# Huangying-Zhan/DF-VO

Measured on AMD Instinct MI355X. Metric: KITTI-odom frames/sec (DF-VO per-pair tracking hot path: monodepth2 + LiteFlowNet fwd/bwd + kp selection + E/H RANSAC + scale), higher is better.
Workload: dtype f32 (f16x3 split products: two f16 planes per operand = 22 mantissa bits, three exact products per term, fp32 accumulate; direct one- / two-channel heads exact fp32)

## Files before the change

### df-vo_amd/capi.py

```python
import ctypes as C
import os

import numpy as np

from . import LIB_PATH


ITER_NOT_RUN = 3
PUSH_NO_FLOW = 1
ERR_RANGE = -4
ERR_EMPTY_SELECTION = -5
ERR_NO_CONSENSUS = -6


class DfvoError(RuntimeError):
    code = None


_lib = None


class Pose2d2dCfg(C.Structure):
    _fields_ = [("fx", C.c_double), ("cx", C.c_double), ("cy", C.c_double), ("reproj_thre", C.c_double),
                ("repeat", C.c_int), ("max_iters", C.c_int), ("KinvT", C.c_double * 9), ("Kinv", C.c_double * 9),
# ... 150 lines not shown
    "dfvo_vis_create": (_i, [_i, _i, C.POINTER(_vp)]),
    "dfvo_vis_destroy": (None, [_vp]),
    "dfvo_vis_cell_rect": (_i, [_vp, _i, _ip]),
    "dfvo_vis_draw_flow": (_i, [_vp, _i, _vp, _i, _i, C.POINTER(C.c_longlong)]),
    "dfvo_vis_draw_map": (_i, [_vp, _i, _vp, _i, _i, _i, _i, _i, _d, C.POINTER(_d)]),
    "dfvo_vis_draw_session": (_i, [_vp, _vp, C.c_longlong, _i, _d, _i, _d, C.POINTER(C.c_longlong), C.POINTER(_d)]),
    "dfvo_vis_session_cells": (_i, [_vp, C.c_longlong, _ip]),
    "dfvo_vis_clear_cell": (_i, [_vp, _i]),
    "dfvo_vis_fetch": (_i, [_vp, _i, _vp]),
    "dfvo_vis_counters": (_i, [_vp, C.POINTER(C.c_longlong)]),
    "dfvo_vis_device_ms": (_i, [_vp, C.POINTER(_f)]),
    "dfvo_vis_flow_rgb": (_i, [_vp, _vp, _i, _i, _vp, C.POINTER(C.c_longlong)]),
    "dfvo_vis_disparity_percentile90": (_i, [_vp, _vp, _i, _i, C.POINTER(_d)]),
    "dfvo_set_conv_precision": (_i, [C.c_char_p]),
    "dfvo_get_conv_precision": (C.c_char_p, []),
    "dfvo_set_sklearn_compat": (_i, [C.c_char_p]),
    "dfvo_f16s_overflow_count": (_i, [C.POINTER(C.c_ulonglong), _i]),
    "dfvo_set_fp32_winograd": (_i, [_i]),
    "dfvo_get_fp32_winograd": (_i, []),
    "dfvo_fp32_winograd_launches": (_i, [C.POINTER(C.c_ulonglong), _i]),
    "dfvo_conv_profile_begin": (_i, []),
    "dfvo_conv_profile_end": (_i, [_vp, _vp, _vp]),
    "dfvo_conv_profile_end_bytes": (_i, [_vp, _vp, _vp, _vp]),
    "dfvo_correlation": (_i, [_vp, _vp, _i, _i, _i, _i, _i, _f, _vp, _vp]),
    "dfvo_backward_warp": (_i, [_vp, _vp, _f, _i, _i, _i, _i, _vp, _vp, _vp, _vp]),
    "dfvo_warp_view": (_i, [_vp, _i, _i, _i, _vp, _i, _i, _f, _i, _i, _i, _i, _vp, _vp, _vp, _i, _i, _i, _i, _vp]),
    "dfvo_correlation_view": (_i, [_vp, _i, _i, _vp, _i, _i, _i, _i, _i, _i, _i, _i, _f, _vp, _i, _vp]),
    "dfvo_flow_mean": (_i, [_vp, _i, _i, _i, _i, _vp, _vp]),
    "dfvo_reg_prep": (_i, [_vp, _vp, _i, _i, _f, _vp, _i, _i, _i, _vp, _vp, _vp, _vp]),
    "dfvo_reg_head": (_i, [_vp, _i, _i, _vp, _i, _i, _vp, _f, _vp, _f, _i, _i, _i, _vp, _i, _i, _vp]),
# ... 202 lines not shown
```

### df-vo_amd/csrc/capi.hip

```cpp
#include "../../include/dfvo_hip.h"

#include <cstdlib>
#include <cstring>
#include <map>
#include <mutex>
#include <utility>
#include <vector>

#include "nets.h"
#include "ops.h"
#include "resize_lanczos.h"
#include "capi_types.h"

namespace dfvo {
static thread_local std::string g_err;
void set_last_error(const std::string& s) { g_err = s; }
const char* last_error() { return g_err.c_str(); }

int ensure_dyn_lds(const void* kernel, size_t bytes) {
    static std::mutex mu;
    static std::map<std::pair<int, const void*>, size_t> configured;
    int dev = 0;
    DFVO_HIP_CHECK(hipGetDevice(&dev));
    std::lock_guard<std::mutex> lock(mu);
// ... 96 lines not shown
    L.ksteps = ksteps;
    L.act = d->act;
    L.act_param = d->act_param;
    static DevArr<float>* const conv2d_ws = new DevArr<float>();
    static std::mutex conv2d_mu;
    std::lock_guard<std::mutex> conv2d_lock(conv2d_mu);
    if (!conv2d_ws->p) (void)conv2d_ws->alloc_zeroed((size_t)4 << 20);
    int rc = run_conv(L, d->N, d->H, d->W, View{d_src0, d->cs0, d->co0}, d->up0, View{d_src1, d->cs1, d->co1}, d_res,
                      d->res_cs, d->res_co, d_dst, d->dst_cs, d->dst_co, d->dst_zero_to, s, nullptr,
                      conv2d_ws->p ? conv2d_ws : nullptr);
    return finish(rc, s);
}

int dfvo_set_conv_precision(const char* name) { return conv_set_precision(name); }
const char* dfvo_get_conv_precision(void) { return conv_get_precision(); }
int dfvo_f16s_overflow_count(unsigned long long* h_count, int reset) { return conv_f16s_overflow_count(h_count, reset); }
int dfvo_set_fp32_winograd(int mode) { return conv_set_fp32_winograd(mode); }
int dfvo_get_fp32_winograd(void) { return conv_fp32_winograd_mode(); }
int dfvo_fp32_winograd_launches(unsigned long long* h_count, int reset) { return conv_fp32_winograd_launches(h_count, reset); }

int dfvo_conv_profile_begin(void) {
    conv_profile_begin();
    return DFVO_OK;
}
int dfvo_conv_profile_end(double* h_ms19, double* h_flops19, int* h_launches19) {
    DFVO_ARG_CHECK(h_ms19 && h_flops19 && h_launches19, "dfvo_conv_profile_end: null argument");
    return conv_profile_end(h_ms19, h_flops19, h_launches19);
}
int dfvo_conv_profile_end_bytes(double* h_ms24, double* h_flops24, int* h_launches24, double* h_bytes24) {
    DFVO_ARG_CHECK(h_ms24 && h_flops24 && h_launches24 && h_bytes24, "dfvo_conv_profile_end_bytes: null argument");
// ... 435 lines not shown
```

### df-vo_amd/csrc/conv.h

```cpp
#pragma once
#include <initializer_list>
#include <string>
#include <type_traits>
#include <vector>

#include "dfvo_common.h"

namespace dfvo {

enum Act { ACT_NONE = 0, ACT_LEAKY = 1, ACT_RELU = 2, ACT_ELU = 3, ACT_SIGMOID = 4 };
enum PadMode { PAD_ZERO = 0, PAD_REFLECT = 1 };

struct ConvParams {
    int N, H, W;
    int Ho, Wo;
    int kh, kw, stride, pad_h, pad_w;
    int pad_mode;
    const float* src0;
    int G0, cs0, co0, up0;
    const float* src1;
    int G1, cs1, co1;
    const float* wp;
    const float* bias;
    const float* wh;
// ... 46 lines not shown
    return (uint32_t)ky | ((uint32_t)kx << 5) | ((uint32_t)valid << 10) | ((uint32_t)src << 11) | ((uint32_t)choff << 16);
}
void conv_build_f16g_table(int c0, int c1, int kh, int kw, std::vector<uint32_t>* tab);
size_t conv_pack_weights_f16g(const float* w_oihw, int cout, int c0, int c1, int kh, int kw, const float* fold_scale,
                              unsigned short* out);
size_t conv_pack_weights_f32g(const float* w_oihw, int cout, int c0, int c1, int kh, int kw, const float* fold_scale, float* out);
size_t conv_wino_f32_weight_floats(int cout, int c0, int c1);
void conv_pack_weights_wino_f32(const float* w_oihw, int cout, int c0, int c1, const float* fold_scale, float* out);
unsigned long long conv_f16s_weights_clamped(bool reset);

constexpr int CONV_NUM_CFGS = 24;
int launch_conv(const ConvParams& p, hipStream_t stream, bool wino_all = false);
bool conv_wino_rule_may_accept(int cout, long long max_pixels);
struct RingShape { bool tc2; int ksp; };
RingShape ring_shape(long long M, int nblk, int steps);

int launch_igemm_f32(const ConvParams& p, hipStream_t stream, int bm, int bn);
int launch_win_f32(const ConvParams& p, hipStream_t stream, int cfg_id);
int launch_head_f32(const ConvParams& p, hipStream_t stream);
bool conv_f16s_ok(const ConvParams& p);
int launch_f16_window(const ConvParams& p, hipStream_t stream);
bool conv_f16g_ok(const ConvParams& p);
int launch_f16g(const ConvParams& p, hipStream_t stream);
unsigned* conv_f16s_overflow_counter();
int conv_f16s_overflow_count(unsigned long long* n, int reset);
bool conv_taps_f16s_ok(const ConvParams& p);
int launch_taps_f16s(const ConvParams& p, hipStream_t stream);
bool conv_f32g_ok(const ConvParams& p);
int launch_f32g(const ConvParams& p, hipStream_t stream);
int conv_fp32_winograd_mode();
// ... 49 lines not shown
```

### df-vo_amd/csrc/conv_dispatch.hip

```cpp
#include "conv.h"

namespace dfvo {

int conv_pick_bn(int cout, long long) {
    if (cout <= 16) return 16;
    if (cout <= 32) return 32;
    if (cout % 128 == 0) return 128;
    if (cout % 64 == 0) return 64;
    if (cout % 32 == 0) return 32;
    return 64;
}

static bool conv_use_head(const ConvParams& p) {
    if (p.cout > 2 || !p.wh) return false;
    if (p.kh != p.kw || p.stride != 1 || p.pad_h != p.kh / 2 || p.pad_w != p.kw / 2) return false;
    if (p.kh != 3 && p.kh != 5 && p.kh != 7) return false;
    return (long long)p.N * p.Ho * p.Wo >= 1024;
}

static bool conv_use_window(const ConvParams& p, int bn) {
    if (p.kh != p.kw || p.stride != 1 || p.pad_h != p.kh / 2 || p.pad_w != p.kw / 2) return false;
    const long long M = (long long)p.N * p.Ho * p.Wo;
    if (p.kh == 3) return bn >= 32 && M >= 30000;
    return (p.kh == 5 || p.kh == 7) && bn == 16 && (p.G0 + p.G1) >= 4 && M >= 8000;
// ... 28 lines not shown
    if (conv_use_head(p) || conv_use_window(p, bn)) return false;
    return (long long)p.N * p.Ho * p.Wo <= 8192;
}

RingShape ring_shape(long long M, int nblk, int steps) {
    const long long mblocks = (M + 31) / 32;
    const long long target = 2048;
    bool tc2 = (nblk % 2) == 0;
    if (tc2 && mblocks * (nblk / 2) * 8 * 2 < target && steps >= 64) tc2 = false;
    const long long tiles = mblocks * (tc2 ? nblk / 2 : nblk);
    int ksp = 1;
    while (ksp < (tc2 ? 8 : 16) && tiles * ksp * 2 <= target && steps >= 4 * ksp * 2) ksp *= 2;
    return {tc2, ksp};
}

int launch_conv(const ConvParams& p, hipStream_t stream, bool wino_all) {
    const long long M = (long long)p.N * p.Ho * p.Wo;
    const int bn = conv_pick_bn(p.cout, M);
    DFVO_ARG_CHECK(p.cout_pad % bn == 0, "launch_conv: cout_pad not a multiple of the N tile");
    DFVO_ARG_CHECK((p.cs0 % 4) == 0 && (p.co0 % 4) == 0, "launch_conv: src0 stride/offset must be multiples of 4");
    DFVO_ARG_CHECK(p.G1 == 0 || ((p.cs1 % 4) == 0 && (p.co1 % 4) == 0), "launch_conv: src1 stride/offset");
    if (conv_use_head(p)) return launch_head_f32(p, stream);
    if (p.wf16 && conv_f16s_ok(p)) return launch_f16_window(p, stream);
    if (conv_f16g_ok(p)) return launch_f16g(p, stream);
    if (conv_wino_applicable(p) && (wino_all || conv_wino_size_rule(p, bn))) return launch_wino(p, stream, conv_window_cfg(p, bn));
    if (conv_f32g_ok(p) && conv_f32g_takes(p, bn)) return launch_f32g(p, stream);
    if (conv_use_window(p, bn)) return launch_win_f32(p, stream, p.kh == 7 ? 16 : (p.kh == 5 ? 17 : conv_window_cfg(p, bn)));
    return launch_igemm_f32(p, stream, conv_pick_bm(p, bn), bn);
}

// ... 2 lines not shown
```

### df-vo_amd/csrc/conv_gemm_f16s.h

```cpp
#pragma once
#include "conv_epi.h"
#include "conv_f16_clamp.h"

namespace dfvo {

typedef unsigned int u32x4 __attribute__((ext_vector_type(4)));
typedef __attribute__((address_space(4))) const u32x4 cu32x4;

template <int WP, int KSP, int TC, int PF = 3, bool RAG = false, int NP = 3>
__global__ __launch_bounds__(64 * WP * KSP) void conv_gemm_f16s_kernel(const ConvParams p) {
    extern __shared__ __attribute__((aligned(16))) float f16g_red[];

    const int t = threadIdx.x, lane = t & 63;
    const int wave = __builtin_amdgcn_readfirstlane(t >> 6);
    const int wp = wave / KSP, wk = wave % KSP;
    const int lp = lane & 31, kb = lane >> 5;
    const int M = p.N * p.Ho * p.Wo;
    const int nb = gridDim.x;
    int bid = blockIdx.x;
    {
        const int q = nb >> 3, r = nb & 7, xcd = bid & 7, k = bid >> 3;
        bid = (xcd < r ? xcd * (q + 1) : r * (q + 1) + (xcd - r) * q) + k;
    }
    const int ny = p.wf16g_cout_pad / (32 * TC);
    const int ytile = bid % ny;
    bid /= ny;
    const int m = (bid * WP + wp) * 32 + lp;
    const bool vm = m < M;
    int iy0, ix0, nimg;
    {
        const int mm = vm ? m : 0;
        nimg = mm / (p.Ho * p.Wo);
        const int rem = mm - nimg * (p.Ho * p.Wo);
        const int oy = rem / p.Wo, ox = rem - oy * p.Wo;
        iy0 = oy * p.stride - p.pad_h;
        ix0 = ox * p.stride - p.pad_w;
    }
    const int n0 = ytile * (32 * TC);
    const int S = p.f16g_steps;
    const int per = (S + KSP - 1) / KSP;
    const int s0 = wk * per < S ? wk * per : S;
    const int s1 = s0 + per < S ? s0 + per : S;

    auto pin = [](int v) { return __builtin_amdgcn_readfirstlane(v); };
    auto pin64 = [](unsigned long long v) {
        const unsigned lo = __builtin_amdgcn_readfirstlane((unsigned)v), hi = __builtin_amdgcn_readfirstlane((unsigned)(v >> 32));
        return ((unsigned long long)hi << 32) | lo;
    };
    const cu32x4* const tab = (const cu32x4*)pin64((unsigned long long)p.f16g_tab);
    const unsigned long long src0 = pin64((unsigned long long)p.src0), src1 = pin64((unsigned long long)(p.G1 ? p.src1 : p.src0));
    const int cs0 = pin(p.cs0), cs1 = pin(p.cs1), co0 = pin(p.co0), co1 = pin(p.co1), up0 = pin(p.up0);
    const int H = pin(p.H), W = pin(p.W), refl = pin(p.pad_mode == PAD_REFLECT ? 1 : 0);
    const int H0 = H >> up0, W0 = W >> up0;
    const unsigned short* const wbase = p.wf16g + ((size_t)n0 * 32 + (kb * 32 + lp) * 8);
    const size_t w_step_stride = (size_t)pin(p.wf16g_cout_pad) * 32;

    f32x4 ra[PF][2];
    unsigned rav = 0;
    h16x8 rw[PF][TC][2];
    const bool fast_addr = !refl && up0 == 0;
    int* const gtab = reinterpret_cast<int*>(f16g_red + (KSP > 1 ? WP * KSP * TC * 16 * 64 : 0));
    if (fast_addr) {
        for (int i = t; i < S * 4; i += 64 * WP * KSP) {
            const unsigned e = p.f16g_tab[i];
            const int ky = e & 31, kx = (e >> 5) & 31;
            const bool s1e = ((e >> 11) & 1u) != 0;
            gtab[2 * i] = (ky * W + kx) * (s1e ? cs1 : cs0) + (int)(e >> 16);
            gtab[2 * i + 1] = (int)(e & 0xfffu);
        }
        __syncthreads();
// ... 168 lines not shown
        if (!vm) continue;
        if (fastq) {
            f32x4 x = v + b + r;
#pragma unroll
            for (int e = 0; e < 4; ++e) x[e] = apply_act(x[e], p.act, p.act_param);
            *reinterpret_cast<f32x4*>(p.dst + (size_t)m * p.dst_cs + p.dst_co + col0) = x;
        } else {
            conv_epilogue_quad(p, (size_t)m, col0, v, vec_ok);
        }
    }
}

template <int WP, int KSP, int TC, int PF = 3, bool RAG = false>
static int launch_f16g_cfg(const ConvParams& p, hipStream_t stream, int cfg_id) {
    const long long M = (long long)p.N * p.Ho * p.Wo;
    dim3 grid((unsigned)(((M + 32 * WP - 1) / (32 * WP)) * (p.wf16g_cout_pad / (32 * TC))), 1, 1);
    const bool fast_addr = p.pad_mode != PAD_REFLECT && p.up0 == 0;
    const size_t lds = (KSP > 1 ? (size_t)WP * KSP * TC * 16 * 64 * sizeof(float) : 0) + (fast_addr ? (size_t)p.f16g_steps * 32 : 0);
    return with_f16_terms(p, [&](auto np) -> int {
        const auto kernel = conv_gemm_f16s_kernel<WP, KSP, TC, PF, RAG, decltype(np)::value>;
        if (lds > 48 * 1024)
            if (int rc_lds = ensure_dyn_lds((const void*)kernel, lds)) return rc_lds;
        ConvProfScope prof(p, stream, cfg_id);
        hipLaunchKernelGGL(kernel, grid, dim3(64 * WP * KSP), lds, stream, p);
        DFVO_HIP_CHECK(hipGetLastError());
        static const std::string variant = conv_variant_name("f16g", {WP, KSP, TC}, RAG ? "rag" : nullptr);
        return prof.done((int)grid.x, TC, KSP * 100 + 1, variant.c_str(), decltype(np)::value);
    });
}

}
```

### df-vo_amd/csrc/conv_gemm_f32g.hip

```cpp
#include "conv.h"
#include "conv_epi.h"

namespace dfvo {

typedef float f32x16g __attribute__((ext_vector_type(16)));
typedef unsigned int u32x4g __attribute__((ext_vector_type(4)));
typedef __attribute__((address_space(4))) const u32x4g cu32x4g;

template <int WP, int KSP, int TC, int PF = 3>
__global__ __launch_bounds__(64 * WP * KSP) void conv_gemm_f32g_kernel(const ConvParams p) {
    extern __shared__ __attribute__((aligned(16))) float f32g_red[];

    const int t = threadIdx.x, lane = t & 63;
    const int wave = __builtin_amdgcn_readfirstlane(t >> 6);
    const int wp = wave / KSP, wk = wave % KSP;
    const int lp = lane & 31, kb = lane >> 5;
    const int M = p.N * p.Ho * p.Wo;
    const int nb = gridDim.x;
    int bid = blockIdx.x;
    {
        const int q = nb >> 3, r = nb & 7, xcd = bid & 7, k = bid >> 3;
        bid = (xcd < r ? xcd * (q + 1) : r * (q + 1) + (xcd - r) * q) + k;
    }
    const int ny = p.wf16g_cout_pad / (32 * TC);
    const int ytile = bid % ny;
    bid /= ny;
    const int m = (bid * WP + wp) * 32 + lp;
    const bool vm = m < M;
    int iy0, ix0, nimg;
    {
        const int mm = vm ? m : 0;
        nimg = mm / (p.Ho * p.Wo);
        const int rem = mm - nimg * (p.Ho * p.Wo);
        const int oy = rem / p.Wo, ox = rem - oy * p.Wo;
        iy0 = oy * p.stride - p.pad_h;
        ix0 = ox * p.stride - p.pad_w;
    }
    const int n0 = ytile * (32 * TC);
    const int S = p.f16g_steps;
    const int per = (S + KSP - 1) / KSP;
    const int s0 = wk * per < S ? wk * per : S;
    const int s1 = s0 + per < S ? s0 + per : S;
// ... 125 lines not shown
            for (int e = 0; e < 4; ++e) x[e] = apply_act(x[e], p.act, p.act_param);
            *reinterpret_cast<f32x4*>(p.dst + (size_t)m * p.dst_cs + p.dst_co + col0) = x;
        } else {
            conv_epilogue_quad(p, (size_t)m, col0, v, vec_ok);
        }
    }
}

bool conv_f32g_ok(const ConvParams& p) {
    return p.wf32g && p.f16g_tab && p.kh <= 31 && p.kw <= 31;
}

template <int WP, int KSP, int TC>
static int launch_f32g_cfg(const ConvParams& p, hipStream_t stream) {
    const long long M = (long long)p.N * p.Ho * p.Wo;
    dim3 grid((unsigned)(((M + 32 * WP - 1) / (32 * WP)) * (p.wf16g_cout_pad / (32 * TC))), 1, 1);
    const size_t lds = KSP > 1 ? (size_t)WP * KSP * TC * 16 * 64 * sizeof(float) : 0;
    if (lds > 48 * 1024)
        if (int rc_lds = ensure_dyn_lds((const void*)conv_gemm_f32g_kernel<WP, KSP, TC>, lds)) return rc_lds;
    ConvProfScope prof(p, stream, KSP == 1 ? 22 : 23);
    hipLaunchKernelGGL((conv_gemm_f32g_kernel<WP, KSP, TC>), grid, dim3(64 * WP * KSP), lds, stream, p);
    DFVO_HIP_CHECK(hipGetLastError());
    static const std::string variant = conv_variant_name("f32g", {WP, KSP, TC});
    return prof.done((int)grid.x, 0, KSP * 100 + 1, variant.c_str());
}

int launch_f32g(const ConvParams& p, hipStream_t stream) {
    const auto [tc2, ksp] = ring_shape((long long)p.N * p.Ho * p.Wo, p.wf16g_cout_pad / 32, p.f16g_steps);
    if (tc2) {
        switch (ksp) {
            case 1: return launch_f32g_cfg<4, 1, 2>(p, stream);
            case 2: return launch_f32g_cfg<2, 2, 2>(p, stream);
            case 4: return launch_f32g_cfg<1, 4, 2>(p, stream);
            default: return launch_f32g_cfg<1, 8, 2>(p, stream);
        }
    }
    switch (ksp) {
        case 1: return launch_f32g_cfg<4, 1, 1>(p, stream);
        case 2: return launch_f32g_cfg<2, 2, 1>(p, stream);
// ... 8 lines not shown
```

### df-vo_amd/csrc/conv_igemm_f32.hip

```cpp
#include "conv.h"

#include <algorithm>

#include "conv_epi.h"

namespace dfvo {

__device__ __forceinline__ void splitk_store(float* dst, f32x4 v) {
    union {
        float f[4];
        unsigned long long u[2];
    } c;
#pragma unroll
    for (int e = 0; e < 4; ++e) c.f[e] = v[e];
    __hip_atomic_store(reinterpret_cast<unsigned long long*>(dst), c.u[0], __ATOMIC_RELAXED, __HIP_MEMORY_SCOPE_AGENT);
    __hip_atomic_store(reinterpret_cast<unsigned long long*>(dst) + 1, c.u[1], __ATOMIC_RELAXED, __HIP_MEMORY_SCOPE_AGENT);
}
__device__ __forceinline__ f32x4 splitk_load(const float* src) {
    union {
        float f[4];
        unsigned long long u[2];
    } c;
    c.u[0] = __hip_atomic_load(reinterpret_cast<const unsigned long long*>(src), __ATOMIC_RELAXED, __HIP_MEMORY_SCOPE_AGENT);
    c.u[1] = __hip_atomic_load(reinterpret_cast<const unsigned long long*>(src) + 1, __ATOMIC_RELAXED, __HIP_MEMORY_SCOPE_AGENT);
// ... 48 lines not shown
    constexpr int BM = WM * TM * 16;
    constexpr int BN = WN * TN * 16;
    constexpr int A_CNT = (BM * 4 + 255) / 256;
    constexpr int B_CNT = (BN * 4 + 255) / 256;
    constexpr int TILE = BM * 16 + BN * 16;
    static_assert(WM * WN == 4, "4 waves per block");
    __shared__ __attribute__((aligned(16))) float lds[2 * TILE];
    __shared__ KGroup ktab[MAX_KGROUPS];

    const int t = threadIdx.x;
    const int lane = t & 63;
    const int wave = t >> 6;
    const int wm = wave / WN;
    const int wn = wave % WN;

    const int nb = gridDim.x;
    int bid = blockIdx.x;
    {
        const int q = nb >> 3, r = nb & 7, xcd = bid & 7, k = bid >> 3;
        bid = (xcd < r ? xcd * (q + 1) : r * (q + 1) + (xcd - r) * q) + k;
    }
    const int m0 = bid * BM;
    const int n0 = blockIdx.y * BN;
    const int M = p.N * p.Ho * p.Wo;
    const int G = p.G0 + p.G1;
    const int taps = p.kh * p.kw;
    const int per = (p.ksteps + (int)gridDim.z - 1) / (int)gridDim.z;
    const int s_begin = (int)blockIdx.z * per;
    const int s_end = s_begin + per < p.ksteps ? s_begin + per : p.ksteps;

    for (int g = s_begin * 4 + t; g < s_end * 4; g += 256) {
        const int tap = g / G;
        const int cg = g - tap * G;
        const int ky = tap / p.kw, kx = tap - ky * p.kw;
        KGroup e;
        const uint32_t valid = tap < taps ? 1u : 0u;
// ... 146 lines not shown
    constexpr int BN = WN * TN * 16;
    constexpr int WIN = WH * WW * PS;
    constexpr int BT = BN * 16;
    constexpr int W_ITEMS = WH * WW * 4;
    constexpr int W_CNT = (W_ITEMS + 255) / 256;
    constexpr int B_CNT = (BN * 4 + 255) / 256;
    static_assert(WM * WN == 4, "4 waves per block");
    __shared__ __attribute__((aligned(16))) float lds[2 * WIN + 2 * BT];
    float* const win = lds;
    float* const bst = lds + 2 * WIN;

    const int t = threadIdx.x, lane = t & 63, wave = t >> 6;
    const int wm = wave / WN, wn = wave % WN;
    const int li = lane & 15, kq = lane >> 4;
    const int tiles_x = (p.Wo + TW - 1) / TW, tiles_y = (p.Ho + TH - 1) / TH;
    const int nb = gridDim.x;
    int bid = blockIdx.x;
    {
        const int q = nb >> 3, r = nb & 7, xcd = bid & 7, k = bid >> 3;
        bid = (xcd < r ? xcd * (q + 1) : r * (q + 1) + (xcd - r) * q) + k;
    }
    const int n = bid / (tiles_y * tiles_x);
    const int trem = bid - n * (tiles_y * tiles_x);
    const int ty0 = (trem / tiles_x) * TH, tx0 = (trem % tiles_x) * TW;
    const int n0 = blockIdx.y * BN;
    const int G = p.G0 + p.G1;
    const int nchunk0 = (p.G0 + 3) >> 2, nchunk1 = (p.G1 + 3) >> 2, nchunks = nchunk0 + nchunk1;
    const int cper = (nchunks + (int)gridDim.z - 1) / (int)gridDim.z;
    const int c_begin = (int)blockIdx.z * cper;
    const int c_end = c_begin + cper < nchunks ? c_begin + cper : nchunks;

    int w_off0[W_CNT], w_off1[W_CNT], w_lds[W_CNT];
    bool w_ok[W_CNT];
#pragma unroll
    for (int r = 0; r < W_CNT; ++r) {
        const int id = t + 256 * r;
// ... 175 lines not shown
    p.dst[(size_t)m * p.dst_cs + p.dst_co + col] = v;
}

typedef __attribute__((address_space(4))) const f32x4 cf32x4;
typedef float f32x2 __attribute__((ext_vector_type(2)));
template <int KS, int CO, int PY = 2>
__global__ __launch_bounds__(256) void conv_head_f32_kernel(const ConvParams p) {
    constexpr int TW = 16, TH = 16 * PY, WH = TH + KS - 1, WW = TW + KS - 1, PS = 12;
    constexpr int WIN = WH * WW * PS;
    constexpr int W_ITEMS = WH * WW * 2;
    constexpr int W_CNT = (W_ITEMS + 255) / 256;
    constexpr int NR = PY + KS - 1;
    __shared__ __attribute__((aligned(16))) float win[WIN];
    const int t = threadIdx.x, tx = t & 15, ty = t >> 4;
    const int tiles_x = (p.Wo + TW - 1) / TW, tiles_y = (p.Ho + TH - 1) / TH;
    const int nb = gridDim.x;
    int bid = blockIdx.x;
    {
        const int q = nb >> 3, r = nb & 7, xcd = bid & 7, k = bid >> 3;
        bid = (xcd < r ? xcd * (q + 1) : r * (q + 1) + (xcd - r) * q) + k;
    }
    const int n = bid / (tiles_y * tiles_x);
    const int trem = bid - n * (tiles_y * tiles_x);
    const int ty0 = (trem / tiles_x) * TH, tx0 = (trem % tiles_x) * TW;
    const int nchunk0 = (p.G0 + 1) >> 1, nchunk1 = (p.G1 + 1) >> 1, nchunks = nchunk0 + nchunk1;

    int w_off0[W_CNT], w_off1[W_CNT], w_lds[W_CNT];
    bool w_ok[W_CNT];
#pragma unroll
    for (int r = 0; r < W_CNT; ++r) {
        const int id = t + 256 * r;
        const int px = id >> 1, q = id & 1;
        const int wy = px / WW, wx = px - wy * WW;
        int iy = ty0 - p.pad_h + wy, ix = tx0 - p.pad_w + wx;
        bool v = id < W_ITEMS;
        if (p.pad_mode == PAD_REFLECT) {
// ... 214 lines not shown
```

### df-vo_amd/csrc/conv_taps_f16s.hip

```cpp
#include "conv.h"
#include "conv_epi.h"
#include "conv_f16_split.h"

namespace dfvo {

typedef unsigned int u32x4t __attribute__((ext_vector_type(4)));
typedef unsigned int u32x2t __attribute__((ext_vector_type(2)));
typedef __attribute__((address_space(4))) const u32x4t cu32x4t;

template <int TH, int TC, int NP = 3, int PF = 3>
__global__ __launch_bounds__(64 * TH) void conv_taps_f16s_kernel(const ConvParams p, int G, int pxd, int wcols, int wrows) {
    extern __shared__ __attribute__((aligned(16))) unsigned char taps_lds[];
    constexpr int NT = 64 * TH;
    const int t = threadIdx.x, lane = t & 63;
    const int wave = __builtin_amdgcn_readfirstlane(t >> 6);
    const int lp = lane & 31, kb = lane >> 5;
    const int tiles_x = (p.Wo + 31) / 32, tiles_y = (p.Ho + TH - 1) / TH;
    const int nb = gridDim.x;
    int bid = blockIdx.x;
    {
        const int q = nb >> 3, r = nb & 7, xcd = bid & 7, k = bid >> 3;
        bid = (xcd < r ? xcd * (q + 1) : r * (q + 1) + (xcd - r) * q) + k;
    }
    const int n = bid / (tiles_y * tiles_x);
    const int trem = bid - n * (tiles_y * tiles_x);
    const int oy0 = (trem / tiles_x) * TH, ox0 = (trem % tiles_x) * 32;
    const int iy0 = oy0 * p.stride - p.pad_h, ix0 = ox0 * p.stride - p.pad_w;

    float amax = 0.f;
    const int npix = wrows * wcols;
    const int zoff = npix * pxd;
    if (t < 4) reinterpret_cast<unsigned*>(taps_lds + zoff)[t] = 0u;
    {
        const int dpx = NT / G, dcg = NT - dpx * G;
        const int dwy = dpx / wcols, dwx = dpx - dwy * wcols;
        int px = t / G, cg = t - px * G;
        int wy = px / wcols, wx = px - wy * wcols;
        constexpr int LB = 4;
// ... 209 lines not shown
```

### df-vo_amd/csrc/conv_win_f16s.h

```cpp
#pragma once
#include "conv_epi.h"
#include "conv_f16_clamp.h"

namespace dfvo {

template <int WC, int WR, int TC, int TR, int NP = 3>
__global__ __launch_bounds__(64 * WC * WR, 2) void conv_win_f16s_kernel(const ConvParams p) {
    constexpr int NT = 64 * WC * WR;
    constexpr int TH = WR * TR, TW = 32, WH = TH + 2, WW = TW + 2, PS = 20;
    constexpr int BN = WC * TC * 32;
    constexpr int WIN = WH * WW * PS;
    constexpr int W_ITEMS = WH * WW * 4;
    constexpr int W_CNT = (W_ITEMS + NT - 1) / NT;
    static_assert(WC * WR == 4 && TC == 1 && W_CNT <= 6, "the one shape left on this skeleton: 4 waves, one cout block per wave");
    __shared__ __attribute__((aligned(16))) float lds[2 * WIN];

    const int t = threadIdx.x, lane = t & 63, wave = t >> 6;
    const int wc = wave / WR, wr = wave % WR;
    const int lp = lane & 31, kb = lane >> 5;
    const int tiles_x = (p.Wo + TW - 1) / TW, tiles_y = (p.Ho + TH - 1) / TH;
    const int nb = gridDim.x;
    int bid = blockIdx.x;
    {
        const int q = nb >> 3, r = nb & 7, xcd = bid & 7, k = bid >> 3;
        bid = (xcd < r ? xcd * (q + 1) : r * (q + 1) + (xcd - r) * q) + k;
    }
    const int n = bid / (tiles_y * tiles_x);
    const int trem = bid - n * (tiles_y * tiles_x);
    const int ty0 = (trem / tiles_x) * TH, tx0 = (trem % tiles_x) * TW;
    const int n0 = blockIdx.y * BN;
    const int nchunk0 = (p.G0 + 3) >> 2, nchunk1 = (p.G1 + 3) >> 2, nchunks = nchunk0 + nchunk1;

    f32x4 rw[W_CNT];
    float amax = 0.f;
    unsigned rwv = 0;
    auto load_window_item = [&](int c, int r) {
        const bool s1 = c >= nchunk0;
        const int cg0 = s1 ? (c - nchunk0) * 4 : c * 4;
        const int Gs = s1 ? p.G1 : p.G0;
        const float* base = s1 ? p.src1 : p.src0;
        const int sh = s1 ? 0 : p.up0;
// ... 161 lines not shown
```

### df-vo_amd/csrc/conv_win_f16s2.h

```cpp
#pragma once
#include <algorithm>
#include <map>
#include <mutex>
#include <tuple>
#include <utility>

#include "conv_win_f16s.h"

namespace dfvo {

template <class F, int... T>
__device__ __forceinline__ void f16s2_static_for_impl(F&& f, std::integer_sequence<int, T...>) {
    (f(std::integral_constant<int, T>{}), ...);
}
template <int N, class F>
__device__ __forceinline__ void f16s2_static_for(F&& f) {
    f16s2_static_for_impl(f, std::make_integer_sequence<int, N>{});
}

template <int WR, int TR>
constexpr int f16s2_lds_floats() {
    return 2 * (((WR * TR + 2) * 34 + 1) * 20);
}

// ... 195 lines not shown
        const int oy = ty0 + wr * TR + j;
        const bool valid = oy < p.Ho && ox < p.Wo;
        const size_t m = valid ? ((size_t)n * p.Ho + oy) * p.Wo + ox : 0;
        conv_epi_row(p, epi, m, valid, [&](int q) {
            f32x4 v;
#pragma unroll
            for (int e = 0; e < 4; ++e) {
                v[e] = am[q >> 2][j][4 * (q & 3) + e];
                if constexpr (NP == 3) v[e] += F16S_LO_UNSCALE * ax[q >> 2][j][4 * (q & 3) + e];
            }
            return v;
        });
    }
}

__device__ __forceinline__ int f16s2_xcd_order(int b, int count) {
    const int q = count >> 3, r = count & 7, xcd = b & 7, k = b >> 3;
    return (xcd < r ? xcd * (q + 1) : r * (q + 1) + (xcd - r) * q) + k;
}

template <int WC, int WR, int TC, int TR, int NP = 3>
__global__ __launch_bounds__(64 * WC * WR, 1) void conv_win_f16s2_kernel(const ConvParams p) {
    constexpr int TH = WR * TR, TW = 32, BN = WC * TC * 32;
    __shared__ __attribute__((aligned(16))) float lds[f16s2_lds_floats<WR, TR>()];
    const int tiles_x = (p.Wo + TW - 1) / TW, tiles_y = (p.Ho + TH - 1) / TH;
    const int bid = f16s2_xcd_order(blockIdx.x, gridDim.x);
    const int n = bid / (tiles_y * tiles_x);
    const int trem = bid - n * (tiles_y * tiles_x);
    conv_win_f16s2_tile<WC, WR, TC, TR, NP>(p, lds, n, (trem / tiles_x) * TH, (trem % tiles_x) * TW, blockIdx.y * BN);
}

template <int WC, int WR, int TC, int TRA, int TRB, int NP = 3>
__global__ __launch_bounds__(64 * WC * WR, 1) void conv_win_f16s2_mix_kernel(const ConvParams p, int rows_a, int na, int na_pad,
                                                                             int nb) {
    constexpr int THA = WR * TRA, THB = WR * TRB, TW = 32, BN = WC * TC * 32;
    constexpr int LDSF = f16s2_lds_floats<WR, TRA>() > f16s2_lds_floats<WR, TRB>() ? f16s2_lds_floats<WR, TRA>() : f16s2_lds_floats<WR, TRB>();
    __shared__ __attribute__((aligned(16))) float lds[LDSF];
    const int tiles_x = (p.Wo + TW - 1) / TW;
    const int b = blockIdx.x;
    if (b < na_pad) {
        const int tiles_y = rows_a / THA;
        const int bid = f16s2_xcd_order(b, na_pad);
        if (bid >= na) return;
        const int n = bid / (tiles_y * tiles_x);
        const int trem = bid - n * (tiles_y * tiles_x);
        conv_win_f16s2_tile<WC, WR, TC, TRA, NP>(p, lds, n, (trem / tiles_x) * THA, (trem % tiles_x) * TW, blockIdx.y * BN);
    } else {
        const int tiles_y = (p.Ho - rows_a + THB - 1) / THB;
        const int bid = f16s2_xcd_order(b - na_pad, nb);
        const int n = bid / (tiles_y * tiles_x);
        const int trem = bid - n * (tiles_y * tiles_x);
        conv_win_f16s2_tile<WC, WR, TC, TRB, NP>(p, lds, n, rows_a + (trem / tiles_x) * THB, (trem % tiles_x) * TW, blockIdx.y * BN);
    }
}

template <int WC, int WR, int TC, int TR>
static int launch_f16s2_cfg(const ConvParams& p, hipStream_t stream, int cfg_id) {
    constexpr int TH = WR * TR, BN = WC * TC * 32;
    const int tiles = p.N * ((p.Ho + TH - 1) / TH) * ((p.Wo + 31) / 32);
    dim3 grid((unsigned)tiles, (unsigned)(p.wf16_cout_pad / BN), 1);
    ConvProfScope prof(p, stream, cfg_id);
    with_f16_terms(p, [&](auto np) {
        hipLaunchKernelGGL((conv_win_f16s2_kernel<WC, WR, TC, TR, decltype(np)::value>), grid, dim3(64 * WC * WR), 0, stream, p);
    });
// ... 100 lines not shown
```

### df-vo_amd/csrc/conv_wino_f32.hip

```cpp
#include "conv.h"

#include <cstdlib>
#include <mutex>

#include "conv_epi.h"
#include "conv_pack_wino_f32.h"

namespace dfvo {

typedef float f32x16 __attribute__((ext_vector_type(16)));

constexpr int WINO_VT = 72;
constexpr int WINO_WW = 18;
constexpr int WINO_PS = 12;
constexpr int WINO_VBUF = 32 * WINO_VT * 4;
constexpr int WINO_RAW = WINO_WW * WINO_WW * WINO_PS;
template <int WN>
constexpr int wino_lds_floats() { return 2 * WINO_VBUF + 2 * (32 * 32 * WN * 4) + WINO_RAW; }

template <int WN>
__global__ __launch_bounds__(128 * WN) void conv_wino_f32_kernel(const ConvParams p, const float* __restrict__ wu, int wcp) {
    constexpr int NT = 128 * WN, BN = 32 * WN;
    constexpr int UBUF = 32 * BN * 4;
    constexpr int W_ITEMS = WINO_WW * WINO_WW * 2;
    constexpr int W_CNT = (W_ITEMS + NT - 1) / NT;
    constexpr int U_CNT = 32 * BN / NT;
    constexpr int T_CNT = 256 / NT;
    extern __shared__ __attribute__((aligned(16))) float wino_lds[];
    float* const vbuf = wino_lds;
    float* const ubuf = wino_lds + 2 * WINO_VBUF;
    float* const raw = ubuf + 2 * UBUF;

    const int t = threadIdx.x, lane = t & 63, wave = t >> 6;
    const int cb = wave % WN, tb = wave / WN;
    const int l31 = lane & 31, hi = lane >> 5;
    const int tiles_x = (p.Wo + 15) / 16, tiles_y = (p.Ho + 15) / 16;
    const int nb = gridDim.x;
    int bid = blockIdx.x;
    {
        const int q = nb >> 3, r = nb & 7, xcd = bid & 7, k = bid >> 3;
        bid = (xcd < r ? xcd * (q + 1) : r * (q + 1) + (xcd - r) * q) + k;
    }
    const int n = bid / (tiles_y * tiles_x);
    const int trem = bid - n * (tiles_y * tiles_x);
    const int ty0 = (trem / tiles_x) * 16, tx0 = (trem % tiles_x) * 16;
    const int n0 = blockIdx.y * BN;
    const int nchunk0 = (p.G0 + 1) >> 1, nchunks = nchunk0 + ((p.G1 + 1) >> 1);

    unsigned w_off0[W_CNT], w_off1[W_CNT];
    int w_lds[W_CNT];
    bool w_ok[W_CNT];
#pragma unroll
    for (int r = 0; r < W_CNT; ++r) {
        const int id = t + NT * r;
        const int px = id >> 1, q = id & 1;
        const int wy = px / WINO_WW, wx = px - wy * WINO_WW;
        int iy = ty0 - 1 + wy, ix = tx0 - 1 + wx;
// ... 197 lines not shown
```

### include/dfvo_hip.h

```cpp
#ifndef DFVO_HIP_H
#define DFVO_HIP_H

#include <stddef.h>
#include <stdint.h>

#ifdef __cplusplus
extern "C" {
#endif

#define DFVO_OK 0
#define DFVO_ERR_HIP (-1)
#define DFVO_ERR_ARG (-2)
#define DFVO_ERR_STATE (-3)
#define DFVO_ERR_RANGE (-4)
#define DFVO_ERR_EMPTY_SELECTION (-5)
#define DFVO_ERR_NO_CONSENSUS (-6)
#define DFVO_ERR_JPEG (-7)

const char* dfvo_last_error(void);
int dfvo_device_count(void);
int dfvo_set_device(int ordinal);
int dfvo_sync_device(void);

int dfvo_malloc(void** d_ptr, size_t bytes);
// ... 8 lines not shown
    int pad_mode;
    int c0, cs0, co0, up0;
    int c1, cs1, co1;
    int cout;
    int act;
    float act_param;
    int res_cs, res_co;
    int dst_cs, dst_co;
    int dst_zero_to;
} dfvo_conv_desc;
int dfvo_conv2d(const dfvo_conv_desc* desc, const float* d_src0, const float* d_src1, const float* h_weight_oihw,
                const float* h_bias, const float* d_res, float* d_dst, void* stream);

int dfvo_set_conv_precision(const char* name);
const char* dfvo_get_conv_precision(void);
int dfvo_set_sklearn_compat(const char* version);
int dfvo_f16s_overflow_count(unsigned long long* h_count, int reset);
int dfvo_set_fp32_winograd(int mode);
int dfvo_get_fp32_winograd(void);
int dfvo_fp32_winograd_launches(unsigned long long* h_count, int reset);
int dfvo_conv_profile_begin(void);
int dfvo_conv_profile_end(double* h_ms24, double* h_flops24, int* h_launches24);
int dfvo_conv_profile_end_bytes(double* h_ms24, double* h_flops24, int* h_launches24, double* h_bytes24);

int dfvo_correlation(const float* d_first, const float* d_second, int N, int H, int W, int C, int stride,
                     float slope, float* d_out, void* stream);

int dfvo_backward_warp(const float* d_src, const float* d_flow, float flow_mult, int N, int H, int W, int C,
                       const float* h_lin_x, const float* h_lin_y, float* d_dst, void* stream);

// ... 458 lines not shown
```

Before: 331.4.

## Partition GEMM conv tiles across XCDs by cout group to cut weight traffic

Adds a tile-ordering scheme for the f16g and f32g GEMM conv kernels. It splits the 8 XCDs into groups, each owning a subset of output-channel tiles, so each XCD's L2 holds only its share of the weights. A byte-cost rule compares weight and activation traffic and picks a split of 1, 2, 4 or 8, applying it only when the estimated traffic drops enough. The change also factors the shared XCD block-order remap into a header and adds an API to force a split. Padded grids can leave some blocks idle, and activations are re-read once per group.

```diff
diff --git a/df-vo_amd/capi.py b/df-vo_amd/capi.py
--- a/df-vo_amd/capi.py
+++ b/df-vo_amd/capi.py
@@ -188,6 +188,7 @@
     "dfvo_vis_disparity_percentile90": (_i, [_vp, _vp, _i, _i, C.POINTER(_d)]),
     "dfvo_set_conv_precision": (_i, [C.c_char_p]),
     "dfvo_get_conv_precision": (C.c_char_p, []),
+    "dfvo_conv_set_tile_split": (_i, [_i]),
     "dfvo_set_sklearn_compat": (_i, [C.c_char_p]),
     "dfvo_f16s_overflow_count": (_i, [C.POINTER(C.c_ulonglong), _i]),
     "dfvo_set_fp32_winograd": (_i, [_i]),
diff --git a/df-vo_amd/csrc/capi.hip b/df-vo_amd/csrc/capi.hip
--- a/df-vo_amd/csrc/capi.hip
+++ b/df-vo_amd/csrc/capi.hip
@@ -134,6 +134,7 @@
 
 int dfvo_set_conv_precision(const char* name) { return conv_set_precision(name); }
 const char* dfvo_get_conv_precision(void) { return conv_get_precision(); }
+int dfvo_conv_set_tile_split(int a) { return conv_set_tile_split(a); }
 int dfvo_f16s_overflow_count(unsigned long long* h_count, int reset) { return conv_f16s_overflow_count(h_count, reset); }
 int dfvo_set_fp32_winograd(int mode) { return conv_set_fp32_winograd(mode); }
 int dfvo_get_fp32_winograd(void) { return conv_fp32_winograd_mode(); }
diff --git a/df-vo_amd/csrc/conv.h b/df-vo_amd/csrc/conv.h
--- a/df-vo_amd/csrc/conv.h
+++ b/df-vo_amd/csrc/conv.h
@@ -84,6 +84,8 @@
 bool conv_wino_rule_may_accept(int cout, long long max_pixels);
 struct RingShape { bool tc2; int ksp; };
 RingShape ring_shape(long long M, int nblk, int steps);
+int ring_tile_split(const ConvParams& p, int ny, double w_bytes);
+int conv_set_tile_split(int a);
 
 int launch_igemm_f32(const ConvParams& p, hipStream_t stream, int bm, int bn);
 int launch_win_f32(const ConvParams& p, hipStream_t stream, int cfg_id);
diff --git a/df-vo_amd/csrc/conv_dispatch.hip b/df-vo_amd/csrc/conv_dispatch.hip
--- a/df-vo_amd/csrc/conv_dispatch.hip
+++ b/df-vo_amd/csrc/conv_dispatch.hip
@@ -1,4 +1,8 @@
 #include "conv.h"
+
+#include <atomic>
+
+#include "conv_tile_order.h"
 
 namespace dfvo {
 
@@ -66,6 +70,22 @@
     return {tc2, ksp};
 }
 
+static std::atomic<int> g_tile_split{0};
+int conv_set_tile_split(int a) {
+    DFVO_ARG_CHECK(a == 0 || a == 1 || a == 2 || a == 4 || a == 8, "dfvo_conv_set_tile_split: expected 0 (the rule), 1, 2, 4 or 8");
+    g_tile_split.store(a);
+    return DFVO_OK;
+}
+int ring_tile_split(const ConvParams& p, int ny, double w_bytes) {
+    int forced = g_tile_split.load(std::memory_order_relaxed);
+    if (forced) {
+        while (!conv_ring_split_legal(forced, ny)) forced >>= 1;
+        return forced;
+    }
+    const double a_bytes = 16.0 * p.N * ((double)(p.H >> p.up0) * (p.W >> p.up0) * p.G0 + (double)p.H * p.W * p.G1);
+    return conv_ring_pick_split(w_bytes, a_bytes, ny);
+}
+
 int launch_conv(const ConvParams& p, hipStream_t stream, bool wino_all) {
     const long long M = (long long)p.N * p.Ho * p.Wo;
     const int bn = conv_pick_bn(p.cout, M);
diff --git a/df-vo_amd/csrc/conv_gemm_f16s.h b/df-vo_amd/csrc/conv_gemm_f16s.h
--- a/df-vo_amd/csrc/conv_gemm_f16s.h
+++ b/df-vo_amd/csrc/conv_gemm_f16s.h
@@ -1,6 +1,7 @@
 #pragma once
 #include "conv_epi.h"
 #include "conv_f16_clamp.h"
+#include "conv_tile_order.h"
 
 namespace dfvo {
 
@@ -8,7 +9,7 @@
 typedef __attribute__((address_space(4))) const u32x4 cu32x4;
 
 template <int WP, int KSP, int TC, int PF = 3, bool RAG = false, int NP = 3>
-__global__ __launch_bounds__(64 * WP * KSP) void conv_gemm_f16s_kernel(const ConvParams p) {
+__global__ __launch_bounds__(64 * WP * KSP) void conv_gemm_f16s_kernel(const ConvParams p, const int split_a) {
     extern __shared__ __attribute__((aligned(16))) float f16g_red[];
 
     const int t = threadIdx.x, lane = t & 63;
@@ -16,16 +17,11 @@
     const int wp = wave / KSP, wk = wave % KSP;
     const int lp = lane & 31, kb = lane >> 5;
     const int M = p.N * p.Ho * p.Wo;
-    const int nb = gridDim.x;
-    int bid = blockIdx.x;
-    {
-        const int q = nb >> 3, r = nb & 7, xcd = bid & 7, k = bid >> 3;
-        bid = (xcd < r ? xcd * (q + 1) : r * (q + 1) + (xcd - r) * q) + k;
-    }
     const int ny = p.wf16g_cout_pad / (32 * TC);
-    const int ytile = bid % ny;
-    bid /= ny;
-    const int m = (bid * WP + wp) * 32 + lp;
+    const ConvTile tile = conv_ring_tile(blockIdx.x, gridDim.x, ny, (M + 32 * WP - 1) / (32 * WP), split_a);
+    if (!tile.valid) return;
+    const int ytile = tile.ytile;
+    const int m = (tile.px * WP + wp) * 32 + lp;
     const bool vm = m < M;
     int iy0, ix0, nimg;
     {
@@ -54,6 +50,7 @@
     const int H0 = H >> up0, W0 = W >> up0;
     const unsigned short* const wbase = p.wf16g + ((size_t)n0 * 32 + (kb * 32 + lp) * 8);
     const size_t w_step_stride = (size_t)pin(p.wf16g_cout_pad) * 32;
+    if (!tile.valid) return;
 
     f32x4 ra[PF][2];
     unsigned rav = 0;
@@ -252,7 +249,9 @@
 template <int WP, int KSP, int TC, int PF = 3, bool RAG = false>
 static int launch_f16g_cfg(const ConvParams& p, hipStream_t stream, int cfg_id) {
     const long long M = (long long)p.N * p.Ho * p.Wo;
-    dim3 grid((unsigned)(((M + 32 * WP - 1) / (32 * WP)) * (p.wf16g_cout_pad / (32 * TC))), 1, 1);
+    const int ny = p.wf16g_cout_pad / (32 * TC);
+    const int split_a = ring_tile_split(p, ny, (double)p.f16g_steps * p.wf16g_cout_pad * 16 * (p.f16_terms == 1 ? 1 : 2) * 2);
+    dim3 grid((unsigned)conv_ring_grid((int)((M + 32 * WP - 1) / (32 * WP)), ny, split_a), 1, 1);
     const bool fast_addr = p.pad_mode != PAD_REFLECT && p.up0 == 0;
     const size_t lds = (KSP > 1 ? (size_t)WP * KSP * TC * 16 * 64 * sizeof(float) : 0) + (fast_addr ? (size_t)p.f16g_steps * 32 : 0);
     return with_f16_terms(p, [&](auto np) -> int {
@@ -260,10 +259,10 @@
         if (lds > 48 * 1024)
             if (int rc_lds = ensure_dyn_lds((const void*)kernel, lds)) return rc_lds;
         ConvProfScope prof(p, stream, cfg_id);
-        hipLaunchKernelGGL(kernel, grid, dim3(64 * WP * KSP), lds, stream, p);
+        hipLaunchKernelGGL(kernel, grid, dim3(64 * WP * KSP), lds, stream, p, split_a);
         DFVO_HIP_CHECK(hipGetLastError());
         static const std::string variant = conv_variant_name("f16g", {WP, KSP, TC}, RAG ? "rag" : nullptr);
-        return prof.done((int)grid.x, TC, KSP * 100 + 1, variant.c_str(), decltype(np)::value);
+        return prof.done((int)grid.x, TC, KSP * 100 + split_a, variant.c_str(), decltype(np)::value);
     });
 }
 
diff --git a/df-vo_amd/csrc/conv_gemm_f32g.hip b/df-vo_amd/csrc/conv_gemm_f32g.hip
--- a/df-vo_amd/csrc/conv_gemm_f32g.hip
+++ b/df-vo_amd/csrc/conv_gemm_f32g.hip
@@ -1,5 +1,6 @@
 #include "conv.h"
 #include "conv_epi.h"
+#include "conv_tile_order.h"
 
 namespace dfvo {
 
@@ -8,7 +9,7 @@
 typedef __attribute__((address_space(4))) const u32x4g cu32x4g;
 
 template <int WP, int KSP, int TC, int PF = 3>
-__global__ __launch_bounds__(64 * WP * KSP) void conv_gemm_f32g_kernel(const ConvParams p) {
+__global__ __launch_bounds__(64 * WP * KSP) void conv_gemm_f32g_kernel(const ConvParams p, const int split_a) {
     extern __shared__ __attribute__((aligned(16))) float f32g_red[];
 
     const int t = threadIdx.x, lane = t & 63;
@@ -16,16 +17,11 @@
     const int wp = wave / KSP, wk = wave % KSP;
     const int lp = lane & 31, kb = lane >> 5;
     const int M = p.N * p.Ho * p.Wo;
-    const int nb = gridDim.x;
-    int bid = blockIdx.x;
-    {
-        const int q = nb >> 3, r = nb & 7, xcd = bid & 7, k = bid >> 3;
-        bid = (xcd < r ? xcd * (q + 1) : r * (q + 1) + (xcd - r) * q) + k;
-    }
     const int ny = p.wf16g_cout_pad / (32 * TC);
-    const int ytile = bid % ny;
-    bid /= ny;
-    const int m = (bid * WP + wp) * 32 + lp;
+    const ConvTile tile = conv_ring_tile(blockIdx.x, gridDim.x, ny, (M + 32 * WP - 1) / (32 * WP), split_a);
+    if (!tile.valid) return;
+    const int ytile = tile.ytile;
+    const int m = (tile.px * WP + wp) * 32 + lp;
     const bool vm = m < M;
     int iy0, ix0, nimg;
     {
@@ -181,15 +177,17 @@
 template <int WP, int KSP, int TC>
 static int launch_f32g_cfg(const ConvParams& p, hipStream_t stream) {
     const long long M = (long long)p.N * p.Ho * p.Wo;
-    dim3 grid((unsigned)(((M + 32 * WP - 1) / (32 * WP)) * (p.wf16g_cout_pad / (32 * TC))), 1, 1);
+    const int ny = p.wf16g_cout_pad / (32 * TC);
+    const int split_a = ring_tile_split(p, ny, (double)p.f16g_steps * p.wf16g_cout_pad * 16 * 4);
+    dim3 grid((unsigned)conv_ring_grid((int)((M + 32 * WP - 1) / (32 * WP)), ny, split_a), 1, 1);
     const size_t lds = KSP > 1 ? (size_t)WP * KSP * TC * 16 * 64 * sizeof(float) : 0;
     if (lds > 48 * 1024)
         if (int rc_lds = ensure_dyn_lds((const void*)conv_gemm_f32g_kernel<WP, KSP, TC>, lds)) return rc_lds;
     ConvProfScope prof(p, stream, KSP == 1 ? 22 : 23);
-    hipLaunchKernelGGL((conv_gemm_f32g_kernel<WP, KSP, TC>), grid, dim3(64 * WP * KSP), lds, stream, p);
+    hipLaunchKernelGGL((conv_gemm_f32g_kernel<WP, KSP, TC>), grid, dim3(64 * WP * KSP), lds, stream, p, split_a);
     DFVO_HIP_CHECK(hipGetLastError());
     static const std::string variant = conv_variant_name("f32g", {WP, KSP, TC});
-    return prof.done((int)grid.x, 0, KSP * 100 + 1, variant.c_str());
+    return prof.done((int)grid.x, 0, KSP * 100 + split_a, variant.c_str());
 }
 
 int launch_f32g(const ConvParams& p, hipStream_t stream) {
diff --git a/df-vo_amd/csrc/conv_igemm_f32.hip b/df-vo_amd/csrc/conv_igemm_f32.hip
--- a/df-vo_amd/csrc/conv_igemm_f32.hip
+++ b/df-vo_amd/csrc/conv_igemm_f32.hip
@@ -3,6 +3,7 @@
 #include <algorithm>
 
 #include "conv_epi.h"
+#include "conv_tile_order.h"
 
 namespace dfvo {
 
@@ -86,12 +87,7 @@
     const int wm = wave / WN;
     const int wn = wave % WN;
 
-    const int nb = gridDim.x;
-    int bid = blockIdx.x;
-    {
-        const int q = nb >> 3, r = nb & 7, xcd = bid & 7, k = bid >> 3;
-        bid = (xcd < r ? xcd * (q + 1) : r * (q + 1) + (xcd - r) * q) + k;
-    }
+    const int bid = conv_xcd_run_order(blockIdx.x, gridDim.x);
     const int m0 = bid * BM;
     const int n0 = blockIdx.y * BN;
     const int M = p.N * p.Ho * p.Wo;
@@ -268,12 +264,7 @@
     const int wm = wave / WN, wn = wave % WN;
     const int li = lane & 15, kq = lane >> 4;
     const int tiles_x = (p.Wo + TW - 1) / TW, tiles_y = (p.Ho + TH - 1) / TH;
-    const int nb = gridDim.x;
-    int bid = blockIdx.x;
-    {
-        const int q = nb >> 3, r = nb & 7, xcd = bid & 7, k = bid >> 3;
-        bid = (xcd < r ? xcd * (q + 1) : r * (q + 1) + (xcd - r) * q) + k;
-    }
+    const int bid = conv_xcd_run_order(blockIdx.x, gridDim.x);
     const int n = bid / (tiles_y * tiles_x);
     const int trem = bid - n * (tiles_y * tiles_x);
     const int ty0 = (trem / tiles_x) * TH, tx0 = (trem % tiles_x) * TW;
@@ -479,12 +470,7 @@
     __shared__ __attribute__((aligned(16))) float win[WIN];
     const int t = threadIdx.x, tx = t & 15, ty = t >> 4;
     const int tiles_x = (p.Wo + TW - 1) / TW, tiles_y = (p.Ho + TH - 1) / TH;
-    const int nb = gridDim.x;
-    int bid = blockIdx.x;
-    {
-        const int q = nb >> 3, r = nb & 7, xcd = bid & 7, k = bid >> 3;
-        bid = (xcd < r ? xcd * (q + 1) : r * (q + 1) + (xcd - r) * q) + k;
-    }
+    const int bid = conv_xcd_run_order(blockIdx.x, gridDim.x);
     const int n = bid / (tiles_y * tiles_x);
     const int trem = bid - n * (tiles_y * tiles_x);
     const int ty0 = (trem / tiles_x) * TH, tx0 = (trem % tiles_x) * TW;
diff --git a/df-vo_amd/csrc/conv_taps_f16s.hip b/df-vo_amd/csrc/conv_taps_f16s.hip
--- a/df-vo_amd/csrc/conv_taps_f16s.hip
+++ b/df-vo_amd/csrc/conv_taps_f16s.hip
@@ -1,6 +1,7 @@
 #include "conv.h"
 #include "conv_epi.h"
 #include "conv_f16_split.h"
+#include "conv_tile_order.h"
 
 namespace dfvo {
 
@@ -16,12 +17,7 @@
     const int wave = __builtin_amdgcn_readfirstlane(t >> 6);
     const int lp = lane & 31, kb = lane >> 5;
     const int tiles_x = (p.Wo + 31) / 32, tiles_y = (p.Ho + TH - 1) / TH;
-    const int nb = gridDim.x;
-    int bid = blockIdx.x;
-    {
-        const int q = nb >> 3, r = nb & 7, xcd = bid & 7, k = bid >> 3;
-        bid = (xcd < r ? xcd * (q + 1) : r * (q + 1) + (xcd - r) * q) + k;
-    }
+    const int bid = conv_xcd_run_order(blockIdx.x, gridDim.x);
     const int n = bid / (tiles_y * tiles_x);
     const int trem = bid - n * (tiles_y * tiles_x);
     const int oy0 = (trem / tiles_x) * TH, ox0 = (trem % tiles_x) * 32;
diff --git a/df-vo_amd/csrc/conv_tile_order.h b/df-vo_amd/csrc/conv_tile_order.h
--- /dev/null
+++ b/df-vo_amd/csrc/conv_tile_order.h
@@ -0,0 +1,64 @@
+#pragma once
+
+#if defined(__HIPCC__) || defined(__CUDACC__)
+#define DFVO_TILE_HD __host__ __device__ __forceinline__
+#else
+#define DFVO_TILE_HD inline
+#endif
+
+namespace dfvo {
+
+DFVO_TILE_HD int conv_xcd_run_order(int b, int count) {
+    const int q = count >> 3, r = count & 7, xcd = b & 7, k = b >> 3;
+    return (xcd < r ? xcd * (q + 1) : r * (q + 1) + (xcd - r) * q) + k;
+}
+
+DFVO_TILE_HD int conv_part_first(int n, int lg, int i) {
+    const int r = n & ((1 << lg) - 1);
+    return i * (n >> lg) + (i < r ? i : r);
+}
+DFVO_TILE_HD int conv_part_len(int n, int lg, int i) { return (n >> lg) + (i < (n & ((1 << lg) - 1)) ? 1 : 0); }
+
+struct ConvTile {
+    int px, ytile;
+    bool valid;
+};
+DFVO_TILE_HD int conv_ring_grid(int nx, int ny, int a) {
+    if (a <= 1) return nx * ny;
+    const int pg = 8 / a;
+    return 8 * ((ny + a - 1) / a) * ((nx + pg - 1) / pg);
+}
+DFVO_TILE_HD ConvTile conv_ring_tile(int b, int grid, int ny, int nx, int a) {
+    int num = conv_xcd_run_order(b, grid), den = ny, x0 = 0, y0 = 0;
+    bool valid = true;
+    if (a > 1) {
+        const int la = a == 8 ? 3 : (a == 4 ? 2 : 1);
+        const int xcd = b & 7, cg = xcd & (a - 1), pg = xcd >> la;
+        y0 = conv_part_first(ny, la, cg);
+        x0 = conv_part_first(nx, 3 - la, pg);
+        den = conv_part_len(ny, la, cg);
+        num = b >> 3;
+        valid = num < den * conv_part_len(nx, 3 - la, pg);
+    }
+    const int quot = num / den;
+    return {x0 + quot, y0 + (num - quot * den), valid};
+}
+
+DFVO_TILE_HD bool conv_ring_split_legal(int a, int ny) { return a == 1 || ((a == 2 || a == 4 || a == 8) && a <= ny); }
+
+DFVO_TILE_HD int conv_ring_pick_split(double w_bytes, double a_bytes, int ny) {
+    const double legacy = w_bytes * 8.0 + a_bytes;
+    int best = 1;
+    double best_cost = legacy;
+    for (int a = 2; a <= 8; a *= 2) {
+        if (!conv_ring_split_legal(a, ny)) break;
+        const double c = w_bytes * (8 / a) + a_bytes * a;
+        if (c < best_cost) {
+            best_cost = c;
+            best = a;
+        }
+    }
+    return best_cost <= 0.75 * legacy ? best : 1;
+}
+
+}
diff --git a/df-vo_amd/csrc/conv_win_f16s.h b/df-vo_amd/csrc/conv_win_f16s.h
--- a/df-vo_amd/csrc/conv_win_f16s.h
+++ b/df-vo_amd/csrc/conv_win_f16s.h
@@ -1,6 +1,7 @@
 #pragma once
 #include "conv_epi.h"
 #include "conv_f16_clamp.h"
+#include "conv_tile_order.h"
 
 namespace dfvo {
 
@@ -19,12 +20,7 @@
     const int wc = wave / WR, wr = wave % WR;
     const int lp = lane & 31, kb = lane >> 5;
     const int tiles_x = (p.Wo + TW - 1) / TW, tiles_y = (p.Ho + TH - 1) / TH;
-    const int nb = gridDim.x;
-    int bid = blockIdx.x;
-    {
-        const int q = nb >> 3, r = nb & 7, xcd = bid & 7, k = bid >> 3;
-        bid = (xcd < r ? xcd * (q + 1) : r * (q + 1) + (xcd - r) * q) + k;
-    }
+    const int bid = conv_xcd_run_order(blockIdx.x, gridDim.x);
     const int n = bid / (tiles_y * tiles_x);
     const int trem = bid - n * (tiles_y * tiles_x);
     const int ty0 = (trem / tiles_x) * TH, tx0 = (trem % tiles_x) * TW;
diff --git a/df-vo_amd/csrc/conv_win_f16s2.h b/df-vo_amd/csrc/conv_win_f16s2.h
--- a/df-vo_amd/csrc/conv_win_f16s2.h
+++ b/df-vo_amd/csrc/conv_win_f16s2.h
@@ -233,17 +233,13 @@
     }
 }
 
-__device__ __forceinline__ int f16s2_xcd_order(int b, int count) {
-    const int q = count >> 3, r = count & 7, xcd = b & 7, k = b >> 3;
-    return (xcd < r ? xcd * (q + 1) : r * (q + 1) + (xcd - r) * q) + k;
-}
 
 template <int WC, int WR, int TC, int TR, int NP = 3>
 __global__ __launch_bounds__(64 * WC * WR, 1) void conv_win_f16s2_kernel(const ConvParams p) {
     constexpr int TH = WR * TR, TW = 32, BN = WC * TC * 32;
     __shared__ __attribute__((aligned(16))) float lds[f16s2_lds_floats<WR, TR>()];
     const int tiles_x = (p.Wo + TW - 1) / TW, tiles_y = (p.Ho + TH - 1) / TH;
-    const int bid = f16s2_xcd_order(blockIdx.x, gridDim.x);
+    const int bid = conv_xcd_run_order(blockIdx.x, gridDim.x);
     const int n = bid / (tiles_y * tiles_x);
     const int trem = bid - n * (tiles_y * tiles_x);
     conv_win_f16s2_tile<WC, WR, TC, TR, NP>(p, lds, n, (trem / tiles_x) * TH, (trem % tiles_x) * TW, blockIdx.y * BN);
@@ -259,14 +255,14 @@
     const int b = blockIdx.x;
     if (b < na_pad) {
         const int tiles_y = rows_a / THA;
-        const int bid = f16s2_xcd_order(b, na_pad);
+        const int bid = conv_xcd_run_order(b, na_pad);
         if (bid >= na) return;
         const int n = bid / (tiles_y * tiles_x);
         const int trem = bid - n * (tiles_y * tiles_x);
         conv_win_f16s2_tile<WC, WR, TC, TRA, NP>(p, lds, n, (trem / tiles_x) * THA, (trem % tiles_x) * TW, blockIdx.y * BN);
     } else {
         const int tiles_y = (p.Ho - rows_a + THB - 1) / THB;
-        const int bid = f16s2_xcd_order(b - na_pad, nb);
+        const int bid = conv_xcd_run_order(b - na_pad, nb);
         const int n = bid / (tiles_y * tiles_x);
         const int trem = bid - n * (tiles_y * tiles_x);
         conv_win_f16s2_tile<WC, WR, TC, TRB, NP>(p, lds, n, rows_a + (trem / tiles_x) * THB, (trem % tiles_x) * TW, blockIdx.y * BN);
diff --git a/df-vo_amd/csrc/conv_wino_f32.hip b/df-vo_amd/csrc/conv_wino_f32.hip
--- a/df-vo_amd/csrc/conv_wino_f32.hip
+++ b/df-vo_amd/csrc/conv_wino_f32.hip
@@ -5,6 +5,7 @@
 
 #include "conv_epi.h"
 #include "conv_pack_wino_f32.h"
+#include "conv_tile_order.h"
 
 namespace dfvo {
 
@@ -35,12 +36,7 @@
     const int cb = wave % WN, tb = wave / WN;
     const int l31 = lane & 31, hi = lane >> 5;
     const int tiles_x = (p.Wo + 15) / 16, tiles_y = (p.Ho + 15) / 16;
-    const int nb = gridDim.x;
-    int bid = blockIdx.x;
-    {
-        const int q = nb >> 3, r = nb & 7, xcd = bid & 7, k = bid >> 3;
-        bid = (xcd < r ? xcd * (q + 1) : r * (q + 1) + (xcd - r) * q) + k;
-    }
+    const int bid = conv_xcd_run_order(blockIdx.x, gridDim.x);
     const int n = bid / (tiles_y * tiles_x);
     const int trem = bid - n * (tiles_y * tiles_x);
     const int ty0 = (trem / tiles_x) * 16, tx0 = (trem % tiles_x) * 16;
diff --git a/include/dfvo_hip.h b/include/dfvo_hip.h
--- a/include/dfvo_hip.h
+++ b/include/dfvo_hip.h
@@ -46,6 +46,7 @@
 
 int dfvo_set_conv_precision(const char* name);
 const char* dfvo_get_conv_precision(void);
+int dfvo_conv_set_tile_split(int a);
 int dfvo_set_sklearn_compat(const char* version);
 int dfvo_f16s_overflow_count(unsigned long long* h_count, int reset);
 int dfvo_set_fp32_winograd(int mode);
```

New measurement: 329.8. About the same (-0.5%).
